# yahoo0742/COSNet

Hardware: AMD Instinct MI355X
Metric: frame-pairs/sec (fwd+bwd) at 473x473 RGBD (higher is better)
Workload: dtype bf16; 1 GPU; RGBDSegmentation_RAA train step (fwd+loss+bwd+SGD), 473x473, batch 4 pairs/GPU; model=RGBDSegmentation_RAA(Bottleneck,[3,4,23,3],[3,4,6,3],1), global_batch=4, parallelism=dp1

## Files before the change

### cosnet_amd/csrc/gemm.hip

```cpp
#include "common.h"
#include "gemm.h"
#include "gemm_dev.h"
#include "../../include/cosnet_hip.h"

#include <type_traits>

namespace {

template <class T> struct Frag;
template <> struct Frag<bf16> { typedef bf16x8 type; };
template <> struct Frag<float> { typedef f32x4 type; };

__device__ __forceinline__ int mc_swz(int k, int granules_per_row) {
  int h = (k & 3) | (((k >> 3) & 1) << 2);
  return (granules_per_row >= 32 ? h : (h & 3)) << 2;
}

__device__ __forceinline__ int mc_swz8(int k) { return (k & 7) ^ ((k >> 5) & 1); }

__device__ __attribute__((aligned(16))) unsigned g_zero16[4];

__device__ __forceinline__ void glds16(const void* src, char* lds_wave_base) {
  __builtin_amdgcn_global_load_lds((const __attribute__((address_space(1))) void*)src,
                                   (__attribute__((address_space(3))) void*)lds_wave_base, 16, 0, 0);
// ... 766 lines not shown
          else if (p.wt)
            __builtin_amdgcn_raw_buffer_store_b128(pk, crs, (int)(((long long)(row - m0) * p.ldc + col) * 2), 0, 16);
          else
            *(u32x4*)dst = pk;
          if (smode) Chunk<bf16>::unpack(pk, v);
        } else {
          if (cmode == 2) {
            f32x4 q0 = *(const f32x4*)dst, q1 = *(const f32x4*)(dst + 4);
#pragma unroll
            for (int e = 0; e < 4; ++e) { v[e] += q0[e]; v[4 + e] += q1[e]; }
          }
          if (p.wt == 4) {
            __builtin_nontemporal_store(*(f32x4*)&v[0], (f32x4*)dst);
            __builtin_nontemporal_store(*(f32x4*)&v[4], (f32x4*)(dst + 4));
          } else if (p.wt) {
            const int off = (int)(((long long)(row - m0) * p.ldc + col) * 4);
            __builtin_amdgcn_raw_buffer_store_b128(__builtin_bit_cast(u32x4, *(f32x4*)&v[0]), crs, off, 0, 16);
            __builtin_amdgcn_raw_buffer_store_b128(__builtin_bit_cast(u32x4, *(f32x4*)&v[4]), crs, off + 16, 0, 16);
          } else {
            *(f32x4*)dst = *(f32x4*)&v[0];
            *(f32x4*)(dst + 4) = *(f32x4*)&v[4];
          }
        }
      } else {
#pragma unroll
        for (int e = 0; e < 8; ++e)
          if (col + e < p.N) {
            store_c<CT>(dst + e, v[e], cmode);
            v[e] = tof((CT)v[e]);
          }
      }
#ifndef CN_EPI_NOACC
      if constexpr (smode == 1) {
        const bool inA = row < segA_end;
#pragma unroll
        for (int e = 0; e < 8; ++e) {
          const float d = (col + e < p.N) ? v[e] - sk[e] : 0.f;
          if (inA) { sa1[e] += d; sa2[e] = fmaf(d, d, sa2[e]); }
          else { sb1[e] += d; sb2[e] = fmaf(d, d, sb2[e]); }
        }
      } else if constexpr (smode == 2) {
        float xv[8];
        if (full) {
          if constexpr (sizeof(CT) == 2) Chunk<bf16>::unpack(xpf[it], xv);
          else { *(u32x4*)&xv[0] = xpf[2 * it]; *(u32x4*)&xv[4] = xpf[2 * it + 1]; }
        } else {
          const CT* xs = (const CT*)p.br_x + (long long)row * p.br_ldx + col;
#pragma unroll
          for (int e = 0; e < 8; ++e) xv[e] = (col + e < p.N) ? tof(xs[e]) : 0.f;
        }
#pragma unroll
        for (int e = 0; e < 8; ++e) {
          float dd = (col + e < p.N && fmaf(xv[e], bk1[e], bsf[e]) > 0.f) ? v[e] : 0.f;
          sa1[e] += dd;
          sa2[e] = fmaf(dd, xv[e] - bmu[e], sa2[e]);
        }
      }
#endif
    }
    __syncthreads();
  }
#ifdef CN_EPI_NORED
  if constexpr (false) {
#else
  if constexpr (smode != 0) {
#endif
    constexpr int NW = NT / 64;
    const int nq = smode == 1 ? 4 : 2;
#pragma unroll
    for (int e = 0; e < 8; ++e) {
#pragma unroll
      for (int o = GPR; o < 64; o <<= 1) {
        sa1[e] += __shfl_xor(sa1[e], o, 64);
        sa2[e] += __shfl_xor(sa2[e], o, 64);
        if (smode == 1) {
          sb1[e] += __shfl_xor(sb1[e], o, 64);
          sb2[e] += __shfl_xor(sb2[e], o, 64);
        }
      }
    }
    float* red = cs;
    if (lane < GPR) {
#pragma unroll
      for (int e = 0; e < 8; ++e) {
        red[(wave * 4 + 0) * BN + c0t + e] = sa1[e];
        red[(wave * 4 + 1) * BN + c0t + e] = sa2[e];
        red[(wave * 4 + 2) * BN + c0t + e] = sb1[e];
        red[(wave * 4 + 3) * BN + c0t + e] = sb2[e];
      }
    }
    __syncthreads();
    float* ws = ((p.ngroup && p.grp.ST[batch]) ? p.grp.ST[batch] : p.st_ws) + (long long)tm * p.N;
    for (int t = tid; t < nq * BN; t += NT) {
      const int q = t / BN, c = t % BN;
      float a = 0.f;
#pragma unroll
      for (int w = 0; w < NW; ++w) a += red[(w * 4 + q) * BN + c];
      if (smode == 2 && q == 1 && n0 + c < p.N) a *= p.br_invstd[n0 + c];
      if (n0 + c < p.N) ws[(long long)(smode == 1 ? q + 1 : q) * p.st_plane + n0 + c] = a;
    }
    if (smode == 1 && tid < GPR) {
#pragma unroll
      for (int e = 0; e < 8; ++e)
        if (n0 + c0t + e < p.N) ws[n0 + c0t + e] = sk[e];
    }
  }
}

struct TileCfg { int bm, bn, wm, wn, s, pp; };
static constexpr TileCfg kCfg[] = {
    {128, 64, 2, 2, 2},
    {128, 128, 2, 2, 2},
    {128, 128, 2, 2, 3},
    {256, 128, 4, 2, 3},
    {128, 256, 2, 4, 3},
    {256, 256, 2, 4, 2},
    {128, 64, 2, 2, 4},
    {128, 128, 2, 2, 4},
    {256, 128, 4, 2, 2},
    {128, 256, 2, 4, 2},
    {256, 256, 4, 2, 2},
    {128, 128, 4, 2, 2},
    {128, 64, 4, 2, 2},
    {128, 128, 4, 2, 3},
    {128, 128, 4, 2, 4},
    {256, 128, 4, 2, 3},
    {128, 64, 4, 2, 4},
    {64, 128, 2, 4, 2},
    {256, 128, 4, 2, 3, 1},
    {128, 256, 2, 4, 3, 1},
    {256, 256, 2, 4, 2, 1},
};
constexpr int kNumCfg = sizeof(kCfg) / sizeof(kCfg[0]);
static int g_force_cfg = -1;

static long long cfg_blocks(int c, const GemmArgs& a, int batch) {
  return (long long)((a.M + kCfg[c].bm - 1) / kCfg[c].bm) * ((a.N + kCfg[c].bn - 1) / kCfg[c].bn) *
         batch * a.nsplit;
}

static long long tiles_of(int c, int M, int N) {
  return (long long)((M + kCfg[c].bm - 1) / kCfg[c].bm) * ((N + kCfg[c].bn - 1) / kCfg[c].bn);
}
static int heuristic_cfg(int M, int N, int K, int bz) {
  if (N <= 64) return 12;
  if (N >= 512 && K >= 2048 && tiles_of(10, M, N) * bz >= 200) return 20;
  if (tiles_of(11, M, N) * bz <= 256 && K >= 512) return 13;
  if (N >= 1024 && K <= 512 && tiles_of(10, M, N) * bz >= 200) return 10;
  return 11;
}

static int pick_cfg(const GemmArgs& a, int batch) {
  if (g_force_cfg >= 0 && g_force_cfg < kNumCfg) return g_force_cfg;
  if (a.cfg >= 0 && a.cfg < kNumCfg) return a.cfg;
  return heuristic_cfg(a.M, a.N, a.K, batch * a.nsplit);
}

template <class T, class CT, int C, int LA, int LB, int EPI = 0>
static int launch_c(const GemmArgs& a, int batch, hipStream_t st) {
  constexpr TileCfg c = kCfg[C];
  dim3 grid((a.M + c.bm - 1) / c.bm, (a.N + c.bn - 1) / c.bn, batch * a.nsplit);
  hipLaunchKernelGGL((gemm_kernel<T, CT, c.bm, c.bn, c.wm, c.wn, c.s, LA, LB, EPI, c.pp>), grid,
                     dim3(c.wm * c.wn * 64), 0, st, a);
  CN_CHECK_LAUNCH();
  return 0;
}

template <class T, int LA, int EPI>
static int launch_epi(const GemmArgs& a, int batch, hipStream_t st) {
  if constexpr (sizeof(T) == 4) {
    if (a.N <= 64 || cfg_blocks(1, a, batch) < 384) return launch_c<T, T, 0, LA, L_KC_DENSE, EPI>(a, batch, st);
    return launch_c<T, T, 1, LA, L_KC_DENSE, EPI>(a, batch, st);
  } else {
    switch (pick_cfg(a, batch)) {
      case 10: return launch_c<T, T, 10, LA, L_KC_DENSE, EPI>(a, batch, st);
      case 11: return launch_c<T, T, 11, LA, L_KC_DENSE, EPI>(a, batch, st);
      case 12: return launch_c<T, T, 12, LA, L_KC_DENSE, EPI>(a, batch, st);
      case 13: return launch_c<T, T, 13, LA, L_KC_DENSE, EPI>(a, batch, st);
      case 18: return launch_c<T, T, 18, LA, L_KC_DENSE, EPI>(a, batch, st);
      case 19: return launch_c<T, T, 19, LA, L_KC_DENSE, EPI>(a, batch, st);
      case 20: return launch_c<T, T, 20, LA, L_KC_DENSE, EPI>(a, batch, st);
      default: return CN_ERR_UNSUPPORTED;
    }
  }
}


template <class T, class CT, int LA, int LB>
static int launch_tile(const GemmArgs& a, int batch, hipStream_t st) {
  if constexpr (sizeof(T) == 2 && sizeof(CT) == 2 && (LA == L_KC_DENSE || LA == L_KC_CONV) &&
                LB == L_KC_DENSE) {
    if (a.c_mode == 2 && !a.row_map && !a.ngroup) {
      switch (pick_cfg(a, batch)) {
        case 10: return launch_c<T, CT, 10, LA, LB, 3>(a, batch, st);
        case 11: return launch_c<T, CT, 11, LA, LB, 3>(a, batch, st);
        case 12: return launch_c<T, CT, 12, LA, LB, 3>(a, batch, st);
        case 13: return launch_c<T, CT, 13, LA, LB, 3>(a, batch, st);
        case 20: return launch_c<T, CT, 20, LA, LB, 3>(a, batch, st);
        default: break;
      }
    }
  }
  if constexpr (sizeof(T) == 4) {
    if (a.N <= 64 || cfg_blocks(1, a, batch) < 384) return launch_c<T, CT, 0, LA, LB>(a, batch, st);
    return launch_c<T, CT, 1, LA, LB>(a, batch, st);
  } else {
    switch (pick_cfg(a, batch)) {
      case 0: return launch_c<T, CT, 0, LA, LB>(a, batch, st);
      case 1: return launch_c<T, CT, 1, LA, LB>(a, batch, st);
      case 2: return launch_c<T, CT, 2, LA, LB>(a, batch, st);
      case 3: return launch_c<T, CT, 3, LA, LB>(a, batch, st);
      case 4: return launch_c<T, CT, 4, LA, LB>(a, batch, st);
      case 5: return launch_c<T, CT, 5, LA, LB>(a, batch, st);
      case 6: return launch_c<T, CT, 6, LA, LB>(a, batch, st);
      case 7: return launch_c<T, CT, 7, LA, LB>(a, batch, st);
      case 8: return launch_c<T, CT, 8, LA, LB>(a, batch, st);
      case 9: return launch_c<T, CT, 9, LA, LB>(a, batch, st);
      case 10: return launch_c<T, CT, 10, LA, LB>(a, batch, st);
      case 11: return launch_c<T, CT, 11, LA, LB>(a, batch, st);
      case 13: return launch_c<T, CT, 13, LA, LB>(a, batch, st);
      case 14: return launch_c<T, CT, 14, LA, LB>(a, batch, st);
      case 15: return launch_c<T, CT, 15, LA, LB>(a, batch, st);
      case 16: return launch_c<T, CT, 16, LA, LB>(a, batch, st);
      case 17: return launch_c<T, CT, 17, LA, LB>(a, batch, st);
      case 18: case 19: case 20: {
        constexpr bool kc = LA != L_MC_DENSE && LA != L_MC_CONV && LB != L_MC_DENSE && LB != L_MC_CONV;
        if constexpr (kc) {
          const int c = pick_cfg(a, batch);
          if (c == 18) return launch_c<T, CT, 18, LA, LB>(a, batch, st);
          if (c == 19) return launch_c<T, CT, 19, LA, LB>(a, batch, st);
          return launch_c<T, CT, 20, LA, LB>(a, batch, st);
        } else {
          if (pick_cfg(a, batch) == 20) return launch_c<T, CT, 10, LA, LB>(a, batch, st);
          return launch_c<T, CT, 11, LA, LB>(a, batch, st);
        }
      }
      default: return launch_c<T, CT, 12, LA, LB>(a, batch, st);
    }
  }
}

template <class T, class CT>
static int launch_conv_g(const GemmArgs& a, int batch, hipStream_t st) {
  if constexpr (sizeof(T) == 4) {
    if (a.N <= 64 || cfg_blocks(1, a, batch) < 384) return launch_c<T, CT, 0, L_KC_CONV_G, L_KC_DENSE>(a, batch, st);
    return launch_c<T, CT, 1, L_KC_CONV_G, L_KC_DENSE>(a, batch, st);
  } else {
    const int c = pick_cfg(a, batch);
    if (c == 12) return launch_c<T, CT, 12, L_KC_CONV_G, L_KC_DENSE>(a, batch, st);
    if (c == 13) return launch_c<T, CT, 13, L_KC_CONV_G, L_KC_DENSE>(a, batch, st);
    return launch_c<T, CT, 11, L_KC_CONV_G, L_KC_DENSE>(a, batch, st);
  }
}

template <class T, class CT>
static int launch_kinds(const GemmArgs& a, int la, int lb, int batch, hipStream_t st) {
#define CN_CASE(A_, B_) \
  if (la == A_ && lb == B_) return launch_tile<T, CT, A_, B_>(a, batch, st);
  if (la == L_KC_CONV_G && lb == L_KC_DENSE) return launch_conv_g<T, CT>(a, batch, st);
  CN_CASE(L_KC_DENSE, L_KC_DENSE)
  CN_CASE(L_KC_CONV, L_KC_DENSE)
  CN_CASE(L_KC_DENSE, L_MC_DENSE)
  CN_CASE(L_MC_DENSE, L_MC_DENSE)
  CN_CASE(L_MC_DENSE, L_MC_CONV)
#undef CN_CASE
  return -10;
}

template <class CT, int LA, class T8 = f8e4m3>
static int launch_f8(const GemmArgs& a, int batch, hipStream_t st) {
  const int c = pick_cfg(a, batch);
  if constexpr (sizeof(CT) == 2 && std::is_same<T8, f8e4m3>::value) {
    if (a.st_mode == 1) {
      if (c == 12) return launch_c<T8, CT, 12, LA, L_KC_DENSE, 1>(a, batch, st);
      if (c == 13) return launch_c<T8, CT, 13, LA, L_KC_DENSE, 1>(a, batch, st);
      return launch_c<T8, CT, 11, LA, L_KC_DENSE, 1>(a, batch, st);
    }
  }
  if (a.st_mode) return CN_ERR_UNSUPPORTED;
  if (c == 12) return launch_c<T8, CT, 12, LA, L_KC_DENSE>(a, batch, st);
  if (c == 13) return launch_c<T8, CT, 13, LA, L_KC_DENSE>(a, batch, st);
  return launch_c<T8, CT, 11, LA, L_KC_DENSE>(a, batch, st);
}

template <int LB>
static int launch_f8_mc(const GemmArgs& a, int batch, hipStream_t st) {
  if (a.cfg == 13) return launch_c<f8e5m2, float, 13, L_MC_DENSE, LB>(a, batch, st);
  return launch_c<f8e5m2, float, 11, L_MC_DENSE, LB>(a, batch, st);
}

static bool buf_ok(int kind, const GemmArgs& a, bool is_a, int esz) {
  const long long ld = is_a ? a.lda : a.ldb;
  const ConvGeom& g = is_a ? a.ga : a.gb;
  const long long kspan = a.nsplit > 1 ? a.k_chunk : a.K;
  if (kind == L_KC_DENSE) return 256 * ld * esz < 0x80000000ll && (long long)a.K * esz < 0xFFFF0000ll;
  if (kind == L_KC_CONV) return (long long)g.N * g.H * g.W * ld * esz < 0x80000000ll;
  if (kind == L_MC_DENSE) return (kspan + 128) * ld * esz < 0xFFFF0000ll && 128 * ld * esz < 0x80000000ll;
  return true;
}

static int g_ws_mode = 1;
static size_t g_ws_launches = 0;
static bool ws_heuristic(const GemmArgs& a) {
  return a.K <= 256 && a.N >= 4 * a.K && a.M >= 8192;
}
static bool ws_eligible(const GemmArgs& a, int dtype, int c_f32, int la, int lb, int batch) {
  if (!g_ws_mode || g_force_cfg >= 0 || a.cfg >= 0) return false;
  if (dtype != DT_BF16 || c_f32 || la != L_KC_DENSE || lb != L_KC_DENSE) return false;
  if (batch != 1 || a.nsplit != 1 || a.row_map || a.ngroup || (a.st_mode && a.st_mode != 4)) return false;
  if (a.st_mode == 4 && a.c_mode != 0) return false;
  if ((a.c_mode != 0 && a.c_mode != 2) || a.bias || a.alpha != 1.f || a.scale_a || a.scale_b) return false;
  if (!cn_gemm_ws_supports(a)) return false;
  return g_ws_mode >= 2 || ws_heuristic(a);
}

int cn_gemm_dispatch(const GemmArgs& a_in, int dtype, int c_f32, int la, int lb, int batch, hipStream_t st) {
  GemmArgs a = a_in;
  a.wt = a.c_mode != 1 && a.c_mode != 3 ? 4 : 0;
  if (a.M <= 0 || a.N <= 0 || batch <= 0) return 0;
  const int esz = (dtype == DT_FP8 || dtype == DT_FP8_E5M2) ? 1 : dtype == DT_BF16 ? 2 : 4;
  const int bk = 128 / esz;
  if (la == L_KC_CONV && (a.ga.C % bk != 0 || !buf_ok(L_KC_CONV, a, true, esz))) la = L_KC_CONV_G;
  if (!buf_ok(la, a, true, esz) || !buf_ok(lb, a, false, esz)) return CN_ERR_SHAPE;
  if (ws_eligible(a, dtype, c_f32, la, lb, batch)) {
    ++g_ws_launches;
    return cn_gemm_ws_launch(a, g_ws_mode == 3 ? 1 : 0, st);
  }
  if (dtype == DT_FP8) {
    if (lb != L_KC_DENSE || a.nsplit != 1) return CN_ERR_UNSUPPORTED;
    if (a.st_mode && (a.st_mode != 1 || batch != 1 || a.row_map || a.c_mode || c_f32)) return CN_ERR_UNSUPPORTED;
    if (la == L_KC_DENSE) return c_f32 ? launch_f8<float, L_KC_DENSE>(a, batch, st) : launch_f8<bf16, L_KC_DENSE>(a, batch, st);
    if (la == L_KC_CONV) return c_f32 ? launch_f8<float, L_KC_CONV>(a, batch, st) : launch_f8<bf16, L_KC_CONV>(a, batch, st);
    if (la == L_KC_CONV_G) return c_f32 ? launch_f8<float, L_KC_CONV_G>(a, batch, st) : launch_f8<bf16, L_KC_CONV_G>(a, batch, st);
    return CN_ERR_UNSUPPORTED;
  }
  if (dtype == DT_FP8_E5M2 && la == L_MC_DENSE) {
    if (!c_f32 || a.st_mode || a.row_map || a.c_mode == 1 || a.c_mode == 2) return CN_ERR_UNSUPPORTED;
    if (lb == L_MC_DENSE) return launch_f8_mc<L_MC_DENSE>(a, batch, st);
    if (lb == L_MC_CONV) return launch_f8_mc<L_MC_CONV>(a, batch, st);
    return CN_ERR_UNSUPPORTED;
  }
  if (dtype == DT_FP8_E5M2) {
    if (lb != L_KC_DENSE || a.st_mode || a.nsplit != 1 || c_f32) return CN_ERR_UNSUPPORTED;
    if (la == L_KC_DENSE) return launch_f8<bf16, L_KC_DENSE, f8e5m2>(a, batch, st);
    if (la == L_KC_CONV) return launch_f8<bf16, L_KC_CONV, f8e5m2>(a, batch, st);
    if (la == L_KC_CONV_G) return launch_f8<bf16, L_KC_CONV_G, f8e5m2>(a, batch, st);
    return CN_ERR_UNSUPPORTED;
  }
  if (a.st_mode) {
    if ((batch != 1 && !(a.ngroup == batch && a.st_mode == 1)) || a.nsplit != 1 || a.row_map || a.c_mode ||
        lb != L_KC_DENSE || (la != L_KC_DENSE && la != L_KC_CONV && la != L_KC_CONV_G))
      return CN_ERR_UNSUPPORTED;
    if (a.st_mode == 4 && (a.ngroup || c_f32 != (dtype == DT_F32) || !a.br_gamma || !a.br_beta ||
                           a.act < 0 || a.act > 2 || (a.act == 2 && !a.prelu)))
      return CN_ERR_UNSUPPORTED;
    if (a.st_mode < 1 || a.st_mode == 3 || a.st_mode > 4) return CN_ERR_UNSUPPORTED;
#define CN_EPI(T_, M_) \
    return la == L_KC_DENSE ? launch_epi<T_, L_KC_DENSE, M_>(a, batch, st) : \
           la == L_KC_CONV ? launch_epi<T_, L_KC_CONV, M_>(a, batch, st) : launch_epi<T_, L_KC_CONV_G, M_>(a, batch, st)
    if (dtype == DT_BF16) {
      if (a.st_mode == 1) CN_EPI(bf16, 1); else if (a.st_mode == 2) CN_EPI(bf16, 2); else CN_EPI(bf16, 4);
    } else {
      if (a.st_mode == 1) CN_EPI(float, 1); else if (a.st_mode == 2) CN_EPI(float, 2); else CN_EPI(float, 4);
    }
#undef CN_EPI
  }
  if (dtype == DT_BF16) {
    return c_f32 ? launch_kinds<bf16, float>(a, la, lb, batch, st)
                 : launch_kinds<bf16, bf16>(a, la, lb, batch, st);
  } else if (dtype == DT_F32) {
    return launch_kinds<float, float>(a, la, lb, batch, st);
  }
  return -11;
}

int cn_gemm_bm(int dtype, int M, int N, int K, int cfg) {
  if (dtype != DT_BF16) return kCfg[1].bm;
  if (g_force_cfg >= 0 && g_force_cfg < kNumCfg) return kCfg[g_force_cfg].bm;
  if (cfg >= 0 && cfg < kNumCfg) return kCfg[cfg].bm;
  return kCfg[heuristic_cfg(M, N, K, 1)].bm;
}

int cn_gemm_pick(int M, int N, int K, int batch_splits) {
  if (g_force_cfg >= 0 && g_force_cfg < kNumCfg) return g_force_cfg;
  return heuristic_cfg(M, N, K, batch_splits);
}

long long cn_gemm_cfg_blocks(int cfg, int M, int N) {
  GemmArgs a = {};
  a.M = M; a.N = N; a.nsplit = 1;
  return cfg_blocks(cfg, a, 1);
}

extern "C" int cn_gemm_force_config(int cfg) {
  if (cfg >= kNumCfg) return -1;
  g_force_cfg = cfg;
  return kNumCfg;
}

extern "C" int cn_gemm_ws_mode(int mode) {
  if (mode < 0 || mode > 3) return -1;
  const int prev = g_ws_mode;
  g_ws_mode = mode;
  return prev;
}

extern "C" size_t cn_gemm_ws_launches(void) { return g_ws_launches; }

template <int G>
__global__ __launch_bounds__(256) void splitk_reduce_k(const float* __restrict__ ws, int nsplit,
                                                       long long slab, long long n4,
                                                       float* __restrict__ out, int accumulate) {
  constexpr int OPB = 256 / G;
  __shared__ f32x4 red[G][OPB];
  const int o = threadIdx.x % OPB, g = threadIdx.x / OPB;
  for (long long base = (long long)blockIdx.x * OPB; base < n4; base += (long long)gridDim.x * OPB) {
    const long long i = base + o;
    f32x4 a = {0.f, 0.f, 0.f, 0.f};
    if (i < n4) {
      int s = g;
      for (; s + 7 * G < nsplit; s += 8 * G) {
        f32x4 v[8];
#pragma unroll
        for (int u = 0; u < 8; ++u) v[u] = *(const f32x4*)(ws + (long long)(s + u * G) * slab + 4 * i);
#pragma unroll
        for (int u = 0; u < 8; ++u) a += v[u];
      }
      for (; s < nsplit; s += G) a += *(const f32x4*)(ws + (long long)s * slab + 4 * i);
    }
    if (G > 1) {
      red[g][o] = a;
      __syncthreads();
      if (g == 0) {
#pragma unroll
        for (int q = 1; q < G; ++q) a += red[q][o];
      }
      __syncthreads();
    }
    if (g == 0 && i < n4) {
      if (accumulate) a += ((const f32x4*)out)[i];
      ((f32x4*)out)[i] = a;
    }
  }
}

int cn_splitk_reduce_impl(const float* ws, int nsplit, long long slab, long long n, float* out,
                          int accumulate, hipStream_t st) {
  if (n % 4 || slab % 4) return -2;
  const long long n4 = n / 4;
  int G = 1;
  while (G < 16 && 2 * G <= nsplit && n4 * G < (512ll << 10)) G *= 2;
  const int opb = 256 / G;
  long long b = (n4 + opb - 1) / opb;
  if (b > 4096) b = 4096;
#define CN_RED(GG) \
  hipLaunchKernelGGL(splitk_reduce_k<GG>, dim3((unsigned)b), dim3(256), 0, st, ws, nsplit, slab, n4, out, accumulate)
  switch (G) {
    case 1: CN_RED(1); break;
    case 2: CN_RED(2); break;
    case 4: CN_RED(4); break;
    case 8: CN_RED(8); break;
    default: CN_RED(16); break;
  }
#undef CN_RED
  CN_CHECK_LAUNCH();
  return 0;
}
```

### cosnet_amd/csrc/gemm_ws.hip

```cpp
#include "common.h"
#include "gemm.h"
#include "gemm_dev.h"
#include "../../include/cosnet_hip.h"

#include <algorithm>
#include <cstdlib>
#include <type_traits>

namespace {

struct WsArgs {
  int M, N;
  const bf16* A; long long lda;
  const bf16* B; long long ldb;
  bf16* C; long long ldc;
  int nslices;
  int wpx;
  int wt;
  const bf16* res; long long ldr;
  const float* scale; const float* shift;
  int act;
};

__device__ __forceinline__ u32x4 load16_asm(const void* p) {
  u32x4 v;
  asm volatile("global_load_dwordx4 %0, %1, off" : "=&v"(v) : "v"(p) : "memory");
  return v;
}

template <int KEEP, bool TIE, int N>
__device__ __forceinline__ void wait_keep(u32x4 (&x)[N]) {
  static_assert(KEEP < 64, "vmcnt is 6 bits");
  asm volatile("s_waitcnt vmcnt(%0)" :: "n"(KEEP) : "memory");
  if constexpr (TIE) {
#pragma unroll
    for (int i = 0; i < N; ++i) asm volatile("" : "+v"(x[i]));
  }
}

template <int KT, int BM, int BN, int WM, int WN, bool MODE2, bool BREG, int FOLD = 0>
__global__ __launch_bounds__(WM * WN * 64, 1) void gemm_ws_kernel(WsArgs p) {
  static_assert(!(MODE2 && FOLD), "the fold stores, it does not accumulate");
  constexpr bool PRE = MODE2 || FOLD == 2;
  constexpr int NT = WM * WN * 64;
  constexpr int BBYTES = KT * BN * 128, ASTG = KT * BM * 128;
  constexpr int TM = BM / WM, TN = BN / WN;
  constexpr int RM = TM / 16, RN = TN / 16;
  constexpr int NCA = BM * 8 / NT, NCB = BN * 8 / NT;
  constexpr int RSTEP = NT / 8;
  constexpr int CSB = TM * TN * 4;
  constexpr int GPR = TN / 8, RPP = 64 / GPR, IT = TM / RPP;
  static_assert(NCA >= 1 && NCA * NT == BM * 8 && NCB * NT == BN * 8, "tiles fill whole chunk rounds");
  static_assert(RSTEP % 8 == 0, "a thread's chunks share row & 7");
  static_assert(IT >= 1 && IT * RPP == TM && (RN & (RN - 1)) == 0, "epilogue passes");
  static_assert(BBYTES + 2 * ASTG + WM * WN * CSB <= 160 * 1024, "LDS budget");
  __shared__ __attribute__((aligned(16))) char smem[BBYTES + 2 * ASTG + WM * WN * CSB];

  const int tid = threadIdx.x, lane = tid & 63;
  const int wave = __builtin_amdgcn_readfirstlane(tid >> 6);
  const int wm = wave / WN, wn = wave % WN;

  const int xcd = blockIdx.x & 7, j = blockIdx.x >> 3;
  const int slice = j % p.nslices;
  const int walker = xcd * p.wpx + j / p.nslices, nwalk = 8 * p.wpx;
  const int n0 = slice * BN;
  const int m16 = (p.M + 15) >> 4;
  const int r0 = (int)((long long)m16 * walker / nwalk) * 16;
  const int r1 = min(p.M, (int)((long long)m16 * (walker + 1) / nwalk) * 16);
  if (r0 >= r1) return;
  const int ntiles = (r1 - r0 + BM - 1) / BM;

  float fsc[FOLD ? 8 : 1], fsh[FOLD ? 8 : 1];
  if constexpr (FOLD != 0) {
    const int fc = n0 + wn * TN + (lane % (TN / 8)) * 8;
    const bool in = fc < p.N;
    const f32x4 z = {0.f, 0.f, 0.f, 0.f};
    const f32x4 s0 = in ? *(const f32x4*)(p.scale + fc) : z, s1 = in ? *(const f32x4*)(p.scale + fc + 4) : z;
    const f32x4 h0 = in ? *(const f32x4*)(p.shift + fc) : z, h1 = in ? *(const f32x4*)(p.shift + fc + 4) : z;
#pragma unroll
    for (int e = 0; e < 4; ++e) { fsc[e] = s0[e]; fsc[4 + e] = s1[e]; fsh[e] = h0[e]; fsh[4 + e] = h1[e]; }
  }

  char* Bs = smem;
  char* As = smem + BBYTES;
  float* cs = (float*)(smem + BBYTES + 2 * ASTG + wave * CSB);
  const int wbase = __builtin_amdgcn_readfirstlane((tid & ~63) * 16);

  const int kcol = ((tid & 7) ^ ((tid >> 3) & 7)) * 8;
  const int rl0 = tid >> 3;

  {
    const __amdgpu_buffer_rsrc_t rb = buf_rsrc(p.B + (long long)n0 * p.ldb);
#pragma unroll
    for (int i = 0; i < NCB; ++i) {
      const int rl = rl0 + RSTEP * i;
      const unsigned voff = n0 + rl < p.N ? (unsigned)((rl * p.ldb + kcol) * 2) : BUF_OOB;
#pragma unroll
      for (int kt = 0; kt < KT; ++kt) blds16(rb, voff, kt * 128, Bs + kt * BN * 128 + wbase + i * NT * 16);
    }
  }
  auto issue_a = [&](int t, char* stg) {
    const int m0 = r0 + t * BM;
    const __amdgpu_buffer_rsrc_t ra = buf_rsrc(p.A + (long long)m0 * p.lda);
#pragma unroll
    for (int i = 0; i < NCA; ++i) {
      const int rl = rl0 + RSTEP * i;
      const unsigned voff = m0 + rl < r1 ? (unsigned)((rl * p.lda + kcol) * 2) : BUF_OOB;
#pragma unroll
      for (int kt = 0; kt < KT; ++kt) blds16(ra, voff, kt * 128, stg + kt * BM * 128 + wbase + i * NT * 16);
    }
  };
  const int erow = wm * TM + lane / GPR, ecol = n0 + wn * TN + (lane % GPR) * 8;
  const bool col_ok = ecol < p.N;
  u32x4 xnx[PRE ? IT : 1], xpf[PRE ? IT : 1];
  const bf16* const pre_base = FOLD == 2 ? p.res : p.C;
  const long long pre_ld = FOLD == 2 ? p.ldr : p.ldc;
  auto fetch_c = [&](int t) {
    const int m0 = r0 + t * BM;
#pragma unroll
    for (int it = 0; it < IT; ++it) {
      const int row = m0 + erow + it * RPP;
      const bf16* src = (row < r1 && col_ok) ? pre_base + (long long)row * pre_ld + ecol : pre_base;
      xnx[it] = load16_asm(src);
    }
  };
  issue_a(0, As);
  if constexpr (PRE) fetch_c(0);
  wait_keep<0, PRE>(xnx);
  raw_barrier();

  bf16x8 breg[BREG ? KT * 2 : 1][RN];
  if constexpr (BREG) {
#pragma unroll
    for (int kt = 0; kt < KT; ++kt)
#pragma unroll
      for (int pc = 0; pc < 2; ++pc)
#pragma unroll
        for (int jj = 0; jj < RN; ++jj)
          breg[kt * 2 + pc][jj] = read_frag_kc_bf16(Bs + kt * BN * 128, wn * TN + jj * 16, pc, lane);
  }

  auto epilogue = [&](int t, auto aux_c, const f32x4 (&acc)[RM][RN]) {
    constexpr int AUX = decltype(aux_c)::value;
    const int m0 = r0 + t * BM;
    const __amdgpu_buffer_rsrc_t rc = buf_rsrc(p.C + (long long)m0 * p.ldc);
    const int g = lane >> 4;
#pragma unroll
    for (int i = 0; i < RM; ++i)
#pragma unroll
      for (int jj = 0; jj < RN; ++jj)
#pragma unroll
        for (int r = 0; r < 4; ++r)
          cs[(i * 16 + 4 * g + r) * TN + (((jj ^ (g & (RN - 1))) << 4) | (lane & 15))] = acc[i][jj][r];
    asm volatile("s_waitcnt lgkmcnt(0)" ::: "memory");
#pragma unroll
    for (int it = 0; it < IT; ++it) {
      const int rr = lane / GPR + it * RPP;
      const int c0 = ((lane % GPR) * 8) ^ ((((rr >> 2) & 3) & (RN - 1)) << 4);
      float v[8];
      *(f32x4*)&v[0] = *(const f32x4*)&cs[rr * TN + c0];
      *(f32x4*)&v[4] = *(const f32x4*)&cs[rr * TN + c0 + 4];
      if constexpr (MODE2) {
        float q[8];
        Chunk<bf16>::unpack(xpf[it], q);
#pragma unroll
        for (int e = 0; e < 8; ++e) v[e] += q[e];
      }
      if constexpr (FOLD != 0) {
        float q[8];
        if constexpr (FOLD == 2) Chunk<bf16>::unpack(xpf[it], q);
#pragma unroll
        for (int e = 0; e < 8; ++e) {
          float u = fmaf(v[e], fsc[e], fsh[e]);
          if constexpr (FOLD == 2) u += q[e];
          v[e] = p.act == 1 ? fmaxf(u, 0.f) : u;
        }
      }
      const int row = erow + it * RPP;
      const unsigned off = (m0 + row < r1 && col_ok) ? (unsigned)(((long long)row * p.ldc + ecol) * 2) : BUF_OOB;
      __builtin_amdgcn_raw_buffer_store_b128(Chunk<bf16>::pack(v), rc, (int)off, 0, AUX);
    }
    asm volatile("" ::: "memory");
  };

#pragma unroll 1
  for (int t = 0; t < ntiles; ++t) {
    char* cur = As + (t & 1) * ASTG;
    if constexpr (PRE) {
#pragma unroll
      for (int it = 0; it < IT; ++it) xpf[it] = xnx[it];
    }
    if (t + 1 < ntiles) {
      issue_a(t + 1, As + ((t + 1) & 1) * ASTG);
      if constexpr (PRE) fetch_c(t + 1);
    }
    f32x4 acc[RM][RN];
#pragma unroll
    for (int i = 0; i < RM; ++i)
#pragma unroll
      for (int jj = 0; jj < RN; ++jj) acc[i][jj] = (f32x4){0.f, 0.f, 0.f, 0.f};
#pragma unroll
    for (int kt = 0; kt < KT; ++kt)
#pragma unroll
      for (int pc = 0; pc < 2; ++pc) {
        bf16x8 af[RM], bfr[RN];
#pragma unroll
        for (int i = 0; i < RM; ++i) af[i] = read_frag_kc_bf16(cur + kt * BM * 128, wm * TM + i * 16, pc, lane);
#pragma unroll
        for (int jj = 0; jj < RN; ++jj) {
          if constexpr (BREG) bfr[jj] = breg[kt * 2 + pc][jj];
          else bfr[jj] = read_frag_kc_bf16(Bs + kt * BN * 128, wn * TN + jj * 16, pc, lane);
        }
#pragma unroll
        for (int i = 0; i < RM; ++i)
#pragma unroll
          for (int jj = 0; jj < RN; ++jj)
            acc[i][jj] = __builtin_amdgcn_mfma_f32_16x16x32_bf16(af[i], bfr[jj], acc[i][jj], 0, 0, 0);
      }
    if (p.wt == 4) epilogue(t, std::integral_constant<int, 2>{}, acc);
    else if (p.wt) epilogue(t, std::integral_constant<int, 16>{}, acc);
    else epilogue(t, std::integral_constant<int, 0>{}, acc);
    if (t + 1 < ntiles) {
      wait_keep<IT, PRE>(xnx);
      raw_barrier();
    }
  }
}

template <int KT, int BM, int BN, int WM, int WN, bool BREG>
int launch_ws(const GemmArgs& a, int cus, int cap, hipStream_t st) {
  WsArgs w;
  w.M = a.M; w.N = a.N;
  w.A = (const bf16*)a.A; w.lda = a.lda;
  w.B = (const bf16*)a.B; w.ldb = a.ldb;
  w.C = (bf16*)a.C; w.ldc = a.ldc;
  w.nslices = (a.N + BN - 1) / BN;
  w.wt = a.wt;
  w.res = (const bf16*)a.br_x; w.ldr = a.br_ldx;
  w.scale = a.br_gamma; w.shift = a.br_beta;
  w.act = a.act;
  const int per_xcd = cus / 8;
  const int want = (int)((((long long)a.M + 15) / 16 + 7) / 8);
  w.wpx = std::min(per_xcd / w.nslices, std::max(want, 1));
  if (cap > 0) w.wpx = std::min(w.wpx, cap);
  if (w.wpx < 1) return CN_ERR_UNSUPPORTED;
  const dim3 grid(8 * w.wpx * w.nslices), block(WM * WN * 64);
  if (a.st_mode == 4 && a.br_x)
    hipLaunchKernelGGL((gemm_ws_kernel<KT, BM, BN, WM, WN, false, BREG, 2>), grid, block, 0, st, w);
  else if (a.st_mode == 4)
    hipLaunchKernelGGL((gemm_ws_kernel<KT, BM, BN, WM, WN, false, BREG, 1>), grid, block, 0, st, w);
  else if (a.c_mode == 2)
    hipLaunchKernelGGL((gemm_ws_kernel<KT, BM, BN, WM, WN, true, BREG>), grid, block, 0, st, w);
  else
    hipLaunchKernelGGL((gemm_ws_kernel<KT, BM, BN, WM, WN, false, BREG>), grid, block, 0, st, w);
  CN_CHECK_LAUNCH();
  return 0;
}

int device_cus() {
  static const int n = [] {
    int dev = 0, v = 0;
    if (hipGetDevice(&dev) != hipSuccess) return 0;
    if (hipDeviceGetAttribute(&v, hipDeviceAttributeMultiprocessorCount, dev) != hipSuccess) return 0;
    return v;
  }();
  return n;
}

int ws_bn(int K) { return K == 512 ? 64 : 128; }

}

bool cn_gemm_ws_supports(const GemmArgs& a) {
  if (a.K != 64 && a.K != 128 && a.K != 256 && a.K != 512) return false;
  if (a.ka_lim < a.K || a.kb_lim < a.K) return false;
  if (a.N % 8 || a.ldc % 8 || (uintptr_t)a.C % 16) return false;
  if (a.lda % 8 || a.ldb % 8 || (uintptr_t)a.A % 16 || (uintptr_t)a.B % 16) return false;
  if (256 * a.ldc * 2 >= 0x80000000ll) return false;
  if (a.st_mode == 4) {
    if (a.act == 2 || (uintptr_t)a.br_gamma % 16 || (uintptr_t)a.br_beta % 16) return false;
    if (a.br_x && (a.br_ldx % 8 || (uintptr_t)a.br_x % 16)) return false;
  }
  const int cus = device_cus();
  return cus >= 8 && (a.N + ws_bn(a.K) - 1) / ws_bn(a.K) <= cus / 8;
}

int cn_gemm_ws_launch(const GemmArgs& a, int walkers_per_xcd, hipStream_t st) {
  const int cus = device_cus();
  switch (a.K) {
    case 64:
      if (a.c_mode == 2) return launch_ws<1, 64, 128, 2, 2, true>(a, cus, walkers_per_xcd, st);
      return launch_ws<1, 128, 128, 4, 2, true>(a, cus, walkers_per_xcd, st);
    case 128: return launch_ws<2, 128, 128, 4, 2, true>(a, cus, walkers_per_xcd, st);
    case 256: return launch_ws<4, 64, 128, 2, 4, true>(a, cus, walkers_per_xcd, st);
    case 512: return launch_ws<8, 32, 64, 2, 2, false>(a, cus, walkers_per_xcd, st);
    default: return CN_ERR_UNSUPPORTED;
  }
}
```

Measured before the change: 137.0 frame-pairs/s.

## Extend weight-stationary GEMM to K=512 by aliasing B tile with A staging

```diff
diff --git a/cosnet_amd/csrc/gemm.hip b/cosnet_amd/csrc/gemm.hip
--- a/cosnet_amd/csrc/gemm.hip
+++ b/cosnet_amd/csrc/gemm.hip
@@ -1092,7 +1092,7 @@
 static int g_ws_mode = 1;
 static size_t g_ws_launches = 0;
 static bool ws_heuristic(const GemmArgs& a) {
-  return a.K <= 256 && a.N >= 4 * a.K && a.M >= 8192;
+  return a.K <= 512 && a.N >= 4 * a.K && a.M >= 8192;
 }
 static bool ws_eligible(const GemmArgs& a, int dtype, int c_f32, int la, int lb, int batch) {
   if (!g_ws_mode || g_force_cfg >= 0 || a.cfg >= 0) return false;
diff --git a/cosnet_amd/csrc/gemm_ws.hip b/cosnet_amd/csrc/gemm_ws.hip
--- a/cosnet_amd/csrc/gemm_ws.hip
+++ b/cosnet_amd/csrc/gemm_ws.hip
@@ -38,7 +38,7 @@
   }
 }
 
-template <int KT, int BM, int BN, int WM, int WN, bool MODE2, bool BREG, int FOLD = 0>
+template <int KT, int BM, int BN, int WM, int WN, bool MODE2, int FOLD = 0>
 __global__ __launch_bounds__(WM * WN * 64, 1) void gemm_ws_kernel(WsArgs p) {
   static_assert(!(MODE2 && FOLD), "the fold stores, it does not accumulate");
   constexpr bool PRE = MODE2 || FOLD == 2;
@@ -53,8 +53,12 @@
   static_assert(NCA >= 1 && NCA * NT == BM * 8 && NCB * NT == BN * 8, "tiles fill whole chunk rounds");
   static_assert(RSTEP % 8 == 0, "a thread's chunks share row & 7");
   static_assert(IT >= 1 && IT * RPP == TM && (RN & (RN - 1)) == 0, "epilogue passes");
-  static_assert(BBYTES + 2 * ASTG + WM * WN * CSB <= 160 * 1024, "LDS budget");
-  __shared__ __attribute__((aligned(16))) char smem[BBYTES + 2 * ASTG + WM * WN * CSB];
+  constexpr int LDS_MAX = 160 * 1024, WALK = 2 * ASTG + WM * WN * CSB;
+  constexpr bool B_OWN = BBYTES + WALK <= LDS_MAX;
+  constexpr int AOFF = B_OWN ? BBYTES : 0;
+  constexpr int SMEM = AOFF + WALK > BBYTES ? AOFF + WALK : BBYTES;
+  static_assert(SMEM <= LDS_MAX, "LDS budget");
+  __shared__ __attribute__((aligned(16))) char smem[SMEM];
 
   const int tid = threadIdx.x, lane = tid & 63;
   const int wave = __builtin_amdgcn_readfirstlane(tid >> 6);
@@ -82,8 +86,8 @@
   }
 
   char* Bs = smem;
-  char* As = smem + BBYTES;
-  float* cs = (float*)(smem + BBYTES + 2 * ASTG + wave * CSB);
+  char* As = smem + AOFF;
+  float* cs = (float*)(smem + AOFF + 2 * ASTG + wave * CSB);
   const int wbase = __builtin_amdgcn_readfirstlane((tid & ~63) * 16);
 
   const int kcol = ((tid & 7) ^ ((tid >> 3) & 7)) * 8;
@@ -124,20 +128,32 @@
       xnx[it] = load16_asm(src);
     }
   };
-  issue_a(0, As);
-  if constexpr (PRE) fetch_c(0);
-  wait_keep<0, PRE>(xnx);
+  if constexpr (B_OWN) {
+    issue_a(0, As);
+    if constexpr (PRE) fetch_c(0);
+  }
+  wait_keep<0, PRE && B_OWN>(xnx);
   raw_barrier();
 
-  bf16x8 breg[BREG ? KT * 2 : 1][RN];
-  if constexpr (BREG) {
-#pragma unroll
-    for (int kt = 0; kt < KT; ++kt)
-#pragma unroll
-      for (int pc = 0; pc < 2; ++pc)
-#pragma unroll
-        for (int jj = 0; jj < RN; ++jj)
-          breg[kt * 2 + pc][jj] = read_frag_kc_bf16(Bs + kt * BN * 128, wn * TN + jj * 16, pc, lane);
+  bf16x8 breg[KT * 2][RN];
+#pragma unroll
+  for (int kt = 0; kt < KT; ++kt)
+#pragma unroll
+    for (int pc = 0; pc < 2; ++pc)
+#pragma unroll
+      for (int jj = 0; jj < RN; ++jj)
+        breg[kt * 2 + pc][jj] = read_frag_kc_bf16(Bs + kt * BN * 128, wn * TN + jj * 16, pc, lane);
+  if constexpr (!B_OWN) {
+    asm volatile("s_waitcnt lgkmcnt(0)" ::: "memory");
+#pragma unroll
+    for (int q = 0; q < KT * 2; ++q)
+#pragma unroll
+      for (int jj = 0; jj < RN; ++jj) asm volatile("" : "+v"(breg[q][jj]));
+    raw_barrier();
+    issue_a(0, As);
+    if constexpr (PRE) fetch_c(0);
+    wait_keep<0, PRE>(xnx);
+    raw_barrier();
   }
 
   auto epilogue = [&](int t, auto aux_c, const f32x4 (&acc)[RM][RN]) {
@@ -203,19 +219,14 @@
     for (int kt = 0; kt < KT; ++kt)
 #pragma unroll
       for (int pc = 0; pc < 2; ++pc) {
-        bf16x8 af[RM], bfr[RN];
+        bf16x8 af[RM];
 #pragma unroll
         for (int i = 0; i < RM; ++i) af[i] = read_frag_kc_bf16(cur + kt * BM * 128, wm * TM + i * 16, pc, lane);
 #pragma unroll
-        for (int jj = 0; jj < RN; ++jj) {
-          if constexpr (BREG) bfr[jj] = breg[kt * 2 + pc][jj];
-          else bfr[jj] = read_frag_kc_bf16(Bs + kt * BN * 128, wn * TN + jj * 16, pc, lane);
-        }
-#pragma unroll
         for (int i = 0; i < RM; ++i)
 #pragma unroll
           for (int jj = 0; jj < RN; ++jj)
-            acc[i][jj] = __builtin_amdgcn_mfma_f32_16x16x32_bf16(af[i], bfr[jj], acc[i][jj], 0, 0, 0);
+            acc[i][jj] = __builtin_amdgcn_mfma_f32_16x16x32_bf16(af[i], breg[kt * 2 + pc][jj], acc[i][jj], 0, 0, 0);
       }
     if (p.wt == 4) epilogue(t, std::integral_constant<int, 2>{}, acc);
     else if (p.wt) epilogue(t, std::integral_constant<int, 16>{}, acc);
@@ -227,7 +238,7 @@
   }
 }
 
-template <int KT, int BM, int BN, int WM, int WN, bool BREG>
+template <int KT, int BM, int BN, int WM, int WN>
 int launch_ws(const GemmArgs& a, int cus, int cap, hipStream_t st) {
   WsArgs w;
   w.M = a.M; w.N = a.N;
@@ -246,13 +257,13 @@
   if (w.wpx < 1) return CN_ERR_UNSUPPORTED;
   const dim3 grid(8 * w.wpx * w.nslices), block(WM * WN * 64);
   if (a.st_mode == 4 && a.br_x)
-    hipLaunchKernelGGL((gemm_ws_kernel<KT, BM, BN, WM, WN, false, BREG, 2>), grid, block, 0, st, w);
+    hipLaunchKernelGGL((gemm_ws_kernel<KT, BM, BN, WM, WN, false, 2>), grid, block, 0, st, w);
   else if (a.st_mode == 4)
-    hipLaunchKernelGGL((gemm_ws_kernel<KT, BM, BN, WM, WN, false, BREG, 1>), grid, block, 0, st, w);
+    hipLaunchKernelGGL((gemm_ws_kernel<KT, BM, BN, WM, WN, false, 1>), grid, block, 0, st, w);
   else if (a.c_mode == 2)
-    hipLaunchKernelGGL((gemm_ws_kernel<KT, BM, BN, WM, WN, true, BREG>), grid, block, 0, st, w);
+    hipLaunchKernelGGL((gemm_ws_kernel<KT, BM, BN, WM, WN, true>), grid, block, 0, st, w);
   else
-    hipLaunchKernelGGL((gemm_ws_kernel<KT, BM, BN, WM, WN, false, BREG>), grid, block, 0, st, w);
+    hipLaunchKernelGGL((gemm_ws_kernel<KT, BM, BN, WM, WN, false>), grid, block, 0, st, w);
   CN_CHECK_LAUNCH();
   return 0;
 }
@@ -267,7 +278,7 @@
   return n;
 }
 
-int ws_bn(int K) { return K == 512 ? 64 : 128; }
+constexpr int WS_BN = 128;
 
 }
 
@@ -282,18 +293,18 @@
     if (a.br_x && (a.br_ldx % 8 || (uintptr_t)a.br_x % 16)) return false;
   }
   const int cus = device_cus();
-  return cus >= 8 && (a.N + ws_bn(a.K) - 1) / ws_bn(a.K) <= cus / 8;
+  return cus >= 8 && (a.N + WS_BN - 1) / WS_BN <= cus / 8;
 }
 
 int cn_gemm_ws_launch(const GemmArgs& a, int walkers_per_xcd, hipStream_t st) {
   const int cus = device_cus();
   switch (a.K) {
     case 64:
-      if (a.c_mode == 2) return launch_ws<1, 64, 128, 2, 2, true>(a, cus, walkers_per_xcd, st);
-      return launch_ws<1, 128, 128, 4, 2, true>(a, cus, walkers_per_xcd, st);
-    case 128: return launch_ws<2, 128, 128, 4, 2, true>(a, cus, walkers_per_xcd, st);
-    case 256: return launch_ws<4, 64, 128, 2, 4, true>(a, cus, walkers_per_xcd, st);
-    case 512: return launch_ws<8, 32, 64, 2, 2, false>(a, cus, walkers_per_xcd, st);
+      if (a.c_mode == 2) return launch_ws<1, 64, 128, 2, 2>(a, cus, walkers_per_xcd, st);
+      return launch_ws<1, 128, 128, 4, 2>(a, cus, walkers_per_xcd, st);
+    case 128: return launch_ws<2, 128, 128, 4, 2>(a, cus, walkers_per_xcd, st);
+    case 256: return launch_ws<4, 64, 128, 2, 4>(a, cus, walkers_per_xcd, st);
+    case 512: return launch_ws<8, 64, 128, 2, 4>(a, cus, walkers_per_xcd, st);
     default: return CN_ERR_UNSUPPORTED;
   }
 }
```

New measurement: 138.2 frame-pairs/s, median of 6. No clear change (+0.9%).
